# sczhou/CodeFormer

Hardware: NVIDIA H100
Metric: faces_per_sec_512x512_batch32 (higher is better)
Workload: dtype f32 (split-fp16 operands on tensor cores, fp32 accumulate)

## Files before the change

### codeformer_b200/csrc/conv_tc.cu

```cuda

#include <cuda.h>
#include <cuda_fp16.h>
#include <cuda_runtime.h>
#include <stdint.h>

#include <stdlib.h>

#include <atomic>
#include <mutex>

#include "conv_tc.cuh"

namespace cfb {

__global__ void tc_absmax_kernel(const float* __restrict__ w, int64_t total, unsigned* __restrict__ slot) {
  float m = 0.f;
  for (int64_t i = (int64_t)blockIdx.x * blockDim.x + threadIdx.x; i < total; i += (int64_t)gridDim.x * blockDim.x)
    m = fmaxf(m, fabsf(w[i]));
#pragma unroll
  for (int o = 16; o > 0; o >>= 1) m = fmaxf(m, __shfl_xor_sync(0xffffffffu, m, o));
  if ((threadIdx.x & 31) == 0) atomicMax(slot, __float_as_uint(m));
}

__global__ void tc_split_weights_kernel(const float* __restrict__ w, __half* __restrict__ hi, __half* __restrict__ lo,
// ... 221 lines not shown
      else if (clock64() - t0 > *(volatile long long*)&g_wait_limit) { mbar_timeout(); aborted = true; break; }
    }
  }
  aborted = __any_sync(0xffffffffu, aborted);
}
__device__ __forceinline__ void mbar_wait(uint32_t bar, uint32_t parity) {
  uint32_t done = 0;
  const long long t0 = clock64();
  while (!done) {
    asm volatile(
        "{\n\t.reg .pred p;\n\t"
        "mbarrier.try_wait.parity.shared::cta.b64 p, [%1], %2, %3;\n\t"
        "selp.u32 %0, 1, 0, p;\n\t}"
        : "=r"(done)
        : "r"(bar), "r"(parity), "r"(0x989680u)
        : "memory");
    if (!done && clock64() - t0 > *(volatile long long*)&g_wait_limit) { mbar_timeout(); break; }
  }
}
__device__ __forceinline__ void tma_load_4d(uint32_t dst, const CUtensorMap* map, uint32_t bar, int c0, int c1, int c2, int c3) {
  asm volatile(
      "cp.async.bulk.tensor.4d.shared::cluster.global.mbarrier::complete_tx::bytes [%0], [%1, {%3, %4, %5, %6}], [%2];"
      ::"r"(dst), "l"(map), "r"(bar), "r"(c0), "r"(c1), "r"(c2), "r"(c3)
      : "memory");
}
__device__ __forceinline__ void tma_load_3d(uint32_t dst, const CUtensorMap* map, uint32_t bar, int c0, int c1, int c2) {
  asm volatile(
      "cp.async.bulk.tensor.3d.shared::cluster.global.mbarrier::complete_tx::bytes [%0], [%1, {%3, %4, %5}], [%2];"
      ::"r"(dst), "l"(map), "r"(bar), "r"(c0), "r"(c1), "r"(c2)
      : "memory");
}
__device__ __forceinline__ bool elect_one() {
  uint32_t pred;
  asm volatile(
      "{\n\t.reg .b32 rx;\n\t.reg .pred px;\n\t"
      "elect.sync rx|px, 0xffffffff;\n\t"
      "selp.b32 %0, 1, 0, px;\n\t}"
      : "=r"(pred));
  return pred != 0;
}

__device__ __forceinline__ uint64_t wg_desc(uint32_t saddr, uint32_t sbo) {
  return (uint64_t)((saddr >> 4) & 0x3FFFu) | ((uint64_t)1 << 16) | ((uint64_t)((sbo >> 4) & 0x3FFFu) << 32) | ((uint64_t)1 << 62);
}
__device__ __forceinline__ void wg_fence() { asm volatile("wgmma.fence.sync.aligned;" ::: "memory"); }
__device__ __forceinline__ void wg_commit() { asm volatile("wgmma.commit_group.sync.aligned;" ::: "memory"); }
__device__ __forceinline__ void wg_wait_all() { asm volatile("wgmma.wait_group.sync.aligned 0;" ::: "memory"); }
__device__ __forceinline__ void wg_mma_64x64(float (&d)[32], uint64_t da, uint64_t db, uint32_t accum) {
  asm volatile(
      "{\n\t.reg .pred p;\n\t"
      "setp.ne.b32 p, %34, 0;\n\t"
      "wgmma.mma_async.sync.aligned.m64n64k16.f32.f16.f16 "
      "{%0, %1, %2, %3, %4, %5, %6, %7, %8, %9, %10, %11, %12, %13, %14, %15, "
      "%16, %17, %18, %19, %20, %21, %22, %23, %24, %25, %26, %27, %28, %29, %30, %31}, %32, %33, p, 1, 1, 0, 0;\n\t}"
      : "+f"(d[0]), "+f"(d[1]), "+f"(d[2]), "+f"(d[3]), "+f"(d[4]), "+f"(d[5]), "+f"(d[6]), "+f"(d[7]), "+f"(d[8]),
        "+f"(d[9]), "+f"(d[10]), "+f"(d[11]), "+f"(d[12]), "+f"(d[13]), "+f"(d[14]), "+f"(d[15]), "+f"(d[16]),
        "+f"(d[17]), "+f"(d[18]), "+f"(d[19]), "+f"(d[20]), "+f"(d[21]), "+f"(d[22]), "+f"(d[23]), "+f"(d[24]),
        "+f"(d[25]), "+f"(d[26]), "+f"(d[27]), "+f"(d[28]), "+f"(d[29]), "+f"(d[30]), "+f"(d[31])
      : "l"(da), "l"(db), "r"(accum)
      : "memory");
}

__device__ __forceinline__ void wg_mma_64x128(float (&d)[64], uint64_t da, uint64_t db, uint32_t accum) {
  asm volatile(
      "{\n\t.reg .pred p;\n\t"
      "setp.ne.b32 p, %66, 0;\n\t"
      "wgmma.mma_async.sync.aligned.m64n128k16.f32.f16.f16 "
      "{%0, %1, %2, %3, %4, %5, %6, %7, %8, %9, %10, %11, %12, %13, %14, %15, "
      "%16, %17, %18, %19, %20, %21, %22, %23, %24, %25, %26, %27, %28, %29, %30, %31, "
      "%32, %33, %34, %35, %36, %37, %38, %39, %40, %41, %42, %43, %44, %45, %46, %47, "
      "%48, %49, %50, %51, %52, %53, %54, %55, %56, %57, %58, %59, %60, %61, %62, %63}, %64, %65, p, 1, 1, 0, 0;\n\t}"
      : "+f"(d[0]), "+f"(d[1]), "+f"(d[2]), "+f"(d[3]), "+f"(d[4]), "+f"(d[5]), "+f"(d[6]), "+f"(d[7]), "+f"(d[8]),
        "+f"(d[9]), "+f"(d[10]), "+f"(d[11]), "+f"(d[12]), "+f"(d[13]), "+f"(d[14]), "+f"(d[15]), "+f"(d[16]),
        "+f"(d[17]), "+f"(d[18]), "+f"(d[19]), "+f"(d[20]), "+f"(d[21]), "+f"(d[22]), "+f"(d[23]), "+f"(d[24]),
        "+f"(d[25]), "+f"(d[26]), "+f"(d[27]), "+f"(d[28]), "+f"(d[29]), "+f"(d[30]), "+f"(d[31]), "+f"(d[32]),
        "+f"(d[33]), "+f"(d[34]), "+f"(d[35]), "+f"(d[36]), "+f"(d[37]), "+f"(d[38]), "+f"(d[39]), "+f"(d[40]),
        "+f"(d[41]), "+f"(d[42]), "+f"(d[43]), "+f"(d[44]), "+f"(d[45]), "+f"(d[46]), "+f"(d[47]), "+f"(d[48]),
        "+f"(d[49]), "+f"(d[50]), "+f"(d[51]), "+f"(d[52]), "+f"(d[53]), "+f"(d[54]), "+f"(d[55]), "+f"(d[56]),
        "+f"(d[57]), "+f"(d[58]), "+f"(d[59]), "+f"(d[60]), "+f"(d[61]), "+f"(d[62]), "+f"(d[63])
      : "l"(da), "l"(db), "r"(accum)
      : "memory");
}
__device__ __forceinline__ void wg_wait_1() { asm volatile("wgmma.wait_group.sync.aligned 1;" ::: "memory"); }

__device__ __forceinline__ bool wg_any(bool v, uint32_t bar_id = 2) {
  uint32_t r;
  asm volatile(
      "{\n\t.reg .pred p, q;\n\t"
      "setp.ne.u32 p, %1, 0;\n\t"
      "bar.red.or.pred q, %2, 128, p;\n\t"
      "selp.u32 %0, 1, 0, q;\n\t}"
      : "=r"(r)
      : "r"((uint32_t)v), "r"(bar_id)
      : "memory");
  return r != 0;
}

__device__ __forceinline__ float ex2_ftz(float x) { float r; asm("ex2.approx.ftz.f32 %0, %1;" : "=f"(r) : "f"(x)); return r; }
__device__ __forceinline__ float rcp_ftz(float x) { float r; asm("rcp.approx.ftz.f32 %0, %1;" : "=f"(r) : "f"(x)); return r; }
__device__ __forceinline__ uint32_t pack_f16x2(float lo, float hi) {
  uint32_t r;
  asm("cvt.rn.f16x2.f32 %0, %1, %2;" : "=r"(r) : "f"(hi), "f"(lo));
  return r;
}
__device__ __forceinline__ float f16_minus_f32(uint32_t h, float c) {
  return __half2float(__ushort_as_half((unsigned short)h)) - c;
}
__device__ __forceinline__ uint4 lds128(uint32_t addr) {
  uint4 v;
  asm volatile("ld.shared.v4.b32 {%0, %1, %2, %3}, [%4];" : "=r"(v.x), "=r"(v.y), "=r"(v.z), "=r"(v.w) : "r"(addr) : "memory");
  return v;
}
__device__ __forceinline__ void sts128(uint32_t addr, const uint4& v) {
  asm volatile("st.shared.v4.b32 [%0], {%1, %2, %3, %4};" ::"r"(addr), "r"(v.x), "r"(v.y), "r"(v.z), "r"(v.w) : "memory");
}
__device__ __forceinline__ float4 lds128f(uint32_t addr) {
  float4 v;
  asm volatile("ld.shared.v4.f32 {%0, %1, %2, %3}, [%4];" : "=f"(v.x), "=f"(v.y), "=f"(v.z), "=f"(v.w) : "r"(addr));
  return v;
}
__device__ __forceinline__ void sts128f(uint32_t addr, float a, float b, float c, float d) {
  asm volatile("st.shared.v4.f32 [%0], {%1, %2, %3, %4};" ::"r"(addr), "f"(a), "f"(b), "f"(c), "f"(d));
}
template <int MODE, bool LO = true>
__device__ __forceinline__ void xf_chunk(const uint4& a, const uint4& b, const float (&sc)[8], const float (&sh)[8], uint4& hv,
                                         uint4& lv, float& amax) {
  const uint32_t raw[8] = {a.x, a.y, a.z, a.w, b.x, b.y, b.z, b.w};
  uint32_t hw[4], lw[4];
#pragma unroll
  for (int q = 0; q < 4; ++q) {
    float y[2];
#pragma unroll
    for (int e = 0; e < 2; ++e) {
      float v = __uint_as_float(raw[2 * q + e]);
      if (MODE >= 1) v = fmaf(v, sc[2 * q + e], sh[2 * q + e]);
      if (MODE == 2) v = v * rcp_ftz(1.f + ex2_ftz(v * -1.4426950408889634f));
      y[e] = v;
    }
    amax = fmaxf(amax, fmaxf(fabsf(y[0]), fabsf(y[1])));
    hw[q] = pack_f16x2(y[0], y[1]);
    if constexpr (LO) {
      const float d0 = f16_minus_f32(hw[q] & 0xffffu, y[0]);
      const float d1 = f16_minus_f32(hw[q] >> 16, y[1]);
      lw[q] = pack_f16x2(d0, d1) ^ 0x80008000u;
    }
  }
  hv = make_uint4(hw[0], hw[1], hw[2], hw[3]);
  if constexpr (LO) lv = make_uint4(lw[0], lw[1], lw[2], lw[3]);
}
template <int MODE, int RPP, int NPASS, int PW, int ROWS, bool LO = true>
__device__ __forceinline__ void xf_patch(uint32_t src_base, uint32_t hi_base, uint32_t lo_base, int c0, int j, int rsub,
                                         const float (&sc)[8], const float (&sh)[8], bool border, int y0, int x0, int Hin,
                                         int Win, float& amax) {
#pragma unroll
  for (int it = 0; it < NPASS; it += 2) {
    uint4 a[2], b[2];
    bool act[2];
#pragma unroll
    for (int u = 0; u < 2; ++u) {
      const int r = rsub + (it + u) * RPP;
      act[u] = (it + u < NPASS) && (r < ROWS);
      if (act[u]) {
        const uint32_t row = src_base + (uint32_t)r * 128u;
        const uint32_t sw = (row >> 7) & 7u;
        a[u] = lds128(row + (((uint32_t)c0 ^ sw) << 4));
        b[u] = lds128(row + (((uint32_t)(c0 + 1) ^ sw) << 4));
      }
    }
    __syncwarp();
#pragma unroll
    for (int u = 0; u < 2; ++u) {
      if (act[u]) {
        const int r = rsub + (it + u) * RPP;
        uint4 hv, lv;
        xf_chunk<MODE, LO>(a[u], b[u], sc, sh, hv, lv, amax);
        if (border) {
          const int py = r / PW, px = r - py * PW;
          if (!((unsigned)(y0 + py) < (unsigned)Hin && (unsigned)(x0 + px) < (unsigned)Win)) {
            hv = make_uint4(0u, 0u, 0u, 0u);
            if constexpr (LO) lv = make_uint4(0u, 0u, 0u, 0u);
          }
        }
        const uint32_t hrow = hi_base + (uint32_t)r * 128u, lrow = lo_base + (uint32_t)r * 128u;
        sts128(hrow + ((((uint32_t)j) ^ ((hrow >> 7) & 7u)) << 4), hv);
        if constexpr (LO) sts128(lrow + ((((uint32_t)j) ^ ((lrow >> 7) & 7u)) << 4), lv);
      }
    }
    __syncwarp();
  }
}

#ifndef CFB_TC_STAMPS
#define CFB_TC_STAMPS 0
#endif
struct TcParams {
  int N, Ho, Wo, Cout;
  int taps, pad, stride;
  int BW, BH;
  int tiles_x, tiles_y;
  int m_tiles, n_tiles;
  int kblocks;
  int chunk;
  int a_c0, b_c0;
  int b_batched;
  int heads;
  int a_c_head, b_c_head;
  int a_img_per_head;
  int b_r_head;
  int out_per_head;
  int o_c_head;
  int up4;
  int PW, PH;
  int Hin, Win;
  int pad_mode;
  int sub;
  int out_pitch, out_c0, cout_valid;
  int res_pitch;
  const float* residual2;
  int res2_pitch;
  float post_scale;
  int fault;
  int xform;
  int a_split;
  const float* in_scale;
  const float* in_shift;
  int in_act;
  const float* bias;
  const float* residual;
  int out_act;
  const float* sft_dec;
  const float* sft_scale;
  float sft_w;
  const float* wscale_inv;
  float* out;
  __half* pl_hi;
  __half* pl_lo;
  float* gn_part;
  int gn_cpg;
  const float* sft_wv;
#if CFB_TC_STAMPS
  long long* dbg;
#endif
};
#if CFB_TC_STAMPS
#define TC_STAMP(i) do { if (p.dbg != nullptr && blockIdx.x == 0) p.dbg[i] = clock64(); } while (0)
#else
#define TC_STAMP(i) do { } while (0)
#endif

constexpr int XF_SKEW = 128;
constexpr int TC_A_BYTES = 128 * 128;

template <int BN>
struct TcCfg {
  static_assert(BN == 64 || BN == 128, "the wgmma engine runs 64- or 128-wide n-tiles");
  static constexpr bool WIDE = BN == 128;
  static constexpr int MMA_WARPS = WIDE ? 8 : 4;
  static constexpr int EPI_WARPS = WIDE ? 4 : 8;
  static constexpr int THREADS = 32 * (MMA_WARPS + 1 + EPI_WARPS);
  static constexpr int B_BYTES = BN * 128;
  static constexpr int STAGE_BYTES = 2 * TC_A_BYTES + 2 * B_BYTES;
  static constexpr int STAGES = 3;
  static constexpr int SLOT_PITCH = BN + 4;
  static constexpr int SLOT_BYTES = 128 * SLOT_PITCH * 4;
  static constexpr int SLOTS = 1;
  static constexpr int STG_BYTES = WIDE ? 0 : 8 * 4096;
  static constexpr int TAIL_BYTES = SLOT_BYTES + 1024  + 512  + STG_BYTES;
  static constexpr int SMEM_BYTES = STAGES * STAGE_BYTES + TAIL_BYTES;
  static constexpr int H_A_PLANE = 23 * 1024;
  static constexpr int H_A_SLOT = 2 * H_A_PLANE;
  static constexpr int H_A_SLOTS = 2;
  static constexpr int H_B_SLOT = 2 * B_BYTES;
  static constexpr int H_B_SLOTS = WIDE ? 2 : 4;
  static constexpr int H_SMEM_BYTES = H_A_SLOTS * H_A_SLOT + H_B_SLOTS * H_B_SLOT + TAIL_BYTES;
  static constexpr int XF_WARPS = WIDE ? 2 : 4;
  static constexpr int XF_THREADS = THREADS + 32 * XF_WARPS + 32;
  static constexpr int X_A_SLOTS = 2;
  static constexpr int X_A_PLANE2 = H_A_PLANE + XF_SKEW;
  static constexpr int X_B_SLOTS = H_B_SLOTS;
  static constexpr int X_SMEM_BYTES = X_A_SLOTS * H_A_SLOT + X_B_SLOTS * H_B_SLOT + TAIL_BYTES;
};

template <int BN, int CPG, bool HALO, bool XF, bool GEN = false, bool K1 = false, bool CM = false, bool SILU = false,
          bool P1 = false>
__global__ void __launch_bounds__(XF ? TcCfg<BN>::XF_THREADS : TcCfg<BN>::THREADS, 1)
conv_tc_kernel(const __grid_constant__ CUtensorMap tmA_hi, const __grid_constant__ CUtensorMap tmA_lo,
               const __grid_constant__ CUtensorMap tmB_hi, const __grid_constant__ CUtensorMap tmB_lo, const TcParams p) {
  static_assert(!XF || HALO, "the fused operand transform exists for the halo engine only");
  static_assert(!GEN || (XF && CPG == 0), "the generalised addressing exists for the fused-transform engine only");
  static_assert(!K1 || (XF && !GEN && CPG == 0), "K1 = fused transform of a 1x1 conv (patch = tile): its own instantiation");
  using Cfg = TcCfg<BN>;
  constexpr bool WIDE = Cfg::WIDE;
  static_assert(!WIDE || (HALO && !GEN && !K1 && CPG != 2), "128-wide tiles exist for the 3x3 / Upsample halo engine");
  static_assert(!CM || (BN == 64 && HALO && !GEN && !K1), "channel-major tiles exist for the 64-channel 3x3 / Upsample halo convs");
  static_assert(!P1 || (!SILU && !K1 && (GEN || WIDE || CM || !HALO)),
                "the single-pass fp16 variant is built for the generalised, 128-wide, channel-major and per-tap engines");
  constexpr int MMA_WARPS = Cfg::MMA_WARPS, EPI_WARPS = Cfg::EPI_WARPS;
  constexpr int A_SLOTS = XF ? Cfg::X_A_SLOTS : Cfg::H_A_SLOTS;
  constexpr int STAGES = Cfg::STAGES;
  constexpr int STAGE_BYTES = Cfg::STAGE_BYTES;
  const int first_tile = (int)blockIdx.x;
  const int tile_step = (int)gridDim.x;
  extern __shared__ uint8_t smem_raw[];
  uint8_t* smem = reinterpret_cast<uint8_t*>((reinterpret_cast<uintptr_t>(smem_raw) + 1023) & ~(uintptr_t)1023);
  constexpr int NRING = HALO ? (XF ? Cfg::X_B_SLOTS : Cfg::H_B_SLOTS) : STAGES;
  constexpr int RING_BYTES = HALO ? Cfg::H_B_SLOT : STAGE_BYTES;
  uint8_t* ring_base = HALO ? smem + A_SLOTS * Cfg::H_A_SLOT : smem;
  float* acc_slot = reinterpret_cast<float*>(ring_base + NRING * RING_BYTES);
  uint64_t* bars = reinterpret_cast<uint64_t*>(ring_base + NRING * RING_BYTES + Cfg::SLOT_BYTES);
  uint64_t* full = bars;
  uint64_t* empty = bars + NRING;
  uint64_t* cfull = bars + 2 * NRING;
  uint64_t* cempty = bars + 2 * NRING + Cfg::SLOTS;
  uint64_t* afull = bars + 2 * NRING + 2 * Cfg::SLOTS;
  uint64_t* aempty = afull + 3;
  uint64_t* araw = aempty + 3;
  uint8_t* stage_buf = reinterpret_cast<uint8_t*>(bars) + 512;

  constexpr int NWARPS = (XF ? Cfg::XF_THREADS : Cfg::THREADS) / 32;
  const int pwarp = __shfl_sync(0xffffffffu, (int)(threadIdx.x >> 5), 0);
  const int ridx = NWARPS - 1 - pwarp;
  const int warp = pwarp < MMA_WARPS ? 1 : (ridx == 0 ? 0 : ridx + 1);
  const int lane = threadIdx.x & 31;
  bool aborted = false;
  if (threadIdx.x == 0) TC_STAMP(0);

  if (warp == 0 && lane == 0) {
    for (int a = 0; a < 3; ++a) {
      mbar_init(smem_u32(afull + a), XF ? Cfg::XF_WARPS : 1);
      mbar_init(smem_u32(aempty + a), MMA_WARPS);
      mbar_init(smem_u32(araw + a), 1);
    }
    asm volatile("prefetch.tensormap [%0];" ::"l"(&tmA_hi) : "memory");
    asm volatile("prefetch.tensormap [%0];" ::"l"(&tmA_lo) : "memory");
    asm volatile("prefetch.tensormap [%0];" ::"l"(&tmB_hi) : "memory");
    asm volatile("prefetch.tensormap [%0];" ::"l"(&tmB_lo) : "memory");
    for (int s = 0; s < NRING; ++s) { mbar_init(smem_u32(full + s), 1); mbar_init(smem_u32(empty + s), MMA_WARPS); }
    for (int a = 0; a < Cfg::SLOTS; ++a) {
      mbar_init(smem_u32(cfull + a), MMA_WARPS);
      mbar_init(smem_u32(cempty + a), EPI_WARPS);
    }
    asm volatile("fence.mbarrier_init.release.cluster;" ::: "memory");
  }
  __syncthreads();
  pdl_launch_dependents();
  pdl_wait();
  if (threadIdx.x == 0) TC_STAMP(1);

  const int total_tiles = p.m_tiles * p.n_tiles;
  const int nk = p.taps * p.kblocks;

  if (warp == 0) {
    {
      int stage = 0;
      uint32_t phase = 0;
      int aslot = 0;
      uint32_t aphase = 0;
      for (int tile = first_tile; tile < total_tiles; tile += tile_step) {
        const int mt = tile / p.n_tiles, nt = tile - mt * p.n_tiles;
        const int mtl = p.up4 ? (mt >> 2) : mt;
        const int par_y = p.up4 ? ((mt & 3) >> 1) : 0, par_x = p.up4 ? (mt & 1) : 0;
        const int per_img = p.tiles_x * p.tiles_y;
        const int n = mtl / per_img;
        const int rem = mtl - n * per_img;
        const int ty = rem / p.tiles_x, tx = rem - ty * p.tiles_x;
        const int y0 = ty * p.BH * p.stride, x0 = tx * p.BW * p.stride;
        if constexpr (HALO) {
          for (int kb = 0; kb < p.kblocks; ++kb) {
            if constexpr (!XF) {
              mbar_wait<500>(smem_u32(aempty + aslot), aphase ^ 1, aborted); if (aborted) goto teardown;
              if (elect_one()) {
                const uint32_t sa = smem_u32(smem + aslot * Cfg::H_A_SLOT);
                const uint32_t ab = smem_u32(afull + aslot);
                mbar_expect_tx(ab, (uint32_t)((P1 ? 1 : 2) * p.PW * p.PH * 128));
                tma_load_4d(sa, &tmA_hi, ab, kb * 64, x0 - p.pad, y0 - p.pad, n);
                if constexpr (!P1) tma_load_4d(sa + Cfg::H_A_PLANE, &tmA_lo, ab, kb * 64, x0 - p.pad, y0 - p.pad, n);
              }
              __syncwarp();
              if (++aslot == A_SLOTS) { aslot = 0; aphase ^= 1; }
            }
            for (int tap = 0; tap < p.taps; ++tap) {
              const int btap = p.up4 ? (mt & 3) * 4 + tap : tap;
              mbar_wait<500>(smem_u32(empty + stage), phase ^ 1, aborted); if (aborted) goto teardown;
              if (elect_one()) {
                if (tile == first_tile && tap == 0 && kb == 0) TC_STAMP(2);
                const uint32_t sb = smem_u32(ring_base + stage * RING_BYTES);
                const uint32_t fb = smem_u32(full + stage);
                const bool drop = p.fault && blockIdx.x == 0 && tile == first_tile && kb == 0 && tap == 0;
                mbar_expect_tx(fb, (uint32_t)(P1 ? Cfg::B_BYTES : Cfg::H_B_SLOT));
                if (!drop) tma_load_3d(sb, &tmB_hi, fb, kb * 64, nt * BN, btap);
                if constexpr (!P1) tma_load_3d(sb + Cfg::B_BYTES, &tmB_lo, fb, kb * 64, nt * BN, btap);
              }
              __syncwarp();
              if (++stage == NRING) { stage = 0; phase ^= 1; }
            }
          }
        } else {
          for (int tap = 0; tap < p.taps; ++tap) {
            int r, s, btap = tap;
            if (p.up4) { r = (tap >> 1) + par_y; s = (tap & 1) + par_x; btap = (mt & 3) * 4 + tap; }
            else { r = (p.taps == 9) ? tap / 3 : 0; s = (p.taps == 9) ? tap - r * 3 : 0; }
            for (int kb = 0; kb < p.kblocks; ++kb) {
              mbar_wait<500>(smem_u32(empty + stage), phase ^ 1, aborted); if (aborted) goto teardown;
              if (elect_one()) {
                if (tile == first_tile && tap == 0 && kb == 0) TC_STAMP(2);
                const uint32_t sa = smem_u32(smem + stage * STAGE_BYTES);
                const int hh = p.heads > 1 ? n % p.heads : 0, nimg = p.heads > 1 ? n / p.heads : n;
                const int a_img = p.a_img_per_head ? n : nimg;
                const int ac = p.a_c0 + hh * p.a_c_head + kb * 64, bc = p.b_c0 + hh * p.b_c_head + kb * 64;
                const int brow = nt * BN + hh * p.b_r_head;
                const int b3 = p.b_batched ? nimg : btap;
                const uint32_t fb = smem_u32(full + stage);
                const bool drop = p.fault && blockIdx.x == 0 && tile == first_tile && kb == 0 && tap == 0;
                mbar_expect_tx(fb, (uint32_t)(P1 ? TC_A_BYTES + Cfg::B_BYTES : Cfg::STAGE_BYTES));
                tma_load_4d(sa, &tmA_hi, fb, ac, x0 + s - p.pad, y0 + r - p.pad, a_img);
                if constexpr (!P1) tma_load_4d(sa + TC_A_BYTES, &tmA_lo, fb, ac, x0 + s - p.pad, y0 + r - p.pad, a_img);
                if (!drop) tma_load_3d(sa + 2 * TC_A_BYTES, &tmB_hi, fb, bc, brow, b3);
                if constexpr (!P1) tma_load_3d(sa + 2 * TC_A_BYTES + Cfg::B_BYTES, &tmB_lo, fb, bc, brow, b3);
              }
              __syncwarp();
              if (++stage == STAGES) { stage = 0; phase ^= 1; }
            }
          }
        }
      }
    }
  } else if (warp == 1) {
    {
      constexpr bool N128 = WIDE || CM;
      constexpr int MH = N128 ? 1 : 2;
      const uint32_t a_sbo = HALO ? (uint32_t)(p.PW * 128) : 1024u;
      const uint32_t a_half = HALO ? (uint32_t)(8 * p.PW * 128) : 8192u;
      const int wq = (int)(threadIdx.x >> 5) & 3;
      const int wg = (int)(threadIdx.x >> 7);
      const uint32_t bar_id = 2u + (uint32_t)wg;
      const uint32_t slot_base = smem_u32(acc_slot);
      int stage = 0;
      uint32_t phase = 0;
      int slot = 0;
      uint32_t slot_phase = 0;
      int aslot = 0;
      uint32_t aphase = 0;
      float acc[MH][N128 ? 64 : 32];
      if constexpr (N128) {
        for (int tile = first_tile; tile < total_tiles; tile += tile_step) {
          const int par = p.up4 ? ((tile / p.n_tiles) & 3) : 0;
          const int par_y = par >> 1, par_x = par & 1;
          for (int c0 = 0; c0 < nk; c0 += p.chunk) {
            const int c1 = min(c0 + p.chunk, nk);
            uint32_t prev_empty = 0, prev_aempty = 0;
            for (int it = c0; it < c1; ++it) {
              const int kb = it / p.taps;
              const int tap = it - kb * p.taps;
              if (tap == 0) {
                mbar_wait(smem_u32(afull + aslot), aphase, aborted);
                if (wg_any(aborted, bar_id)) { wg_wait_all(); aborted = true; goto teardown; }
              }
              int r = (p.taps == 9) ? tap / 3 : 0;
              int sft = (p.taps == 9) ? tap - r * 3 : 0;
              if (p.up4) { r = (tap >> 1) + par_y; sft = (tap & 1) + par_x; }
              const uint32_t a_hi0 = smem_u32(smem + aslot * Cfg::H_A_SLOT) + (uint32_t)((r * p.PW + sft) * 128) +
                                     (uint32_t)wg * a_half;
              const uint32_t a_lo0 = a_hi0 + (uint32_t)(XF ? Cfg::X_A_PLANE2 : Cfg::H_A_PLANE);
              const uint32_t bsm = smem_u32(ring_base + stage * RING_BYTES);
              mbar_wait(smem_u32(full + stage), phase, aborted);
              if (wg_any(aborted, bar_id)) { wg_wait_all(); aborted = true; goto teardown; }
              wg_fence();
#pragma unroll
              for (int k = 0; k < 4; ++k) {
                const uint64_t db_hi = wg_desc(bsm + 32 * k, 1024u), db_lo = wg_desc(bsm + Cfg::B_BYTES + 32 * k, 1024u);
                const uint64_t da_hi = wg_desc(a_hi0 + 32 * k, a_sbo), da_lo = wg_desc(a_lo0 + 32 * k, a_sbo);
                if constexpr (P1 && CM) {
                  wg_mma_64x128(acc[0], db_hi, da_hi, (it == c0 && k == 0) ? 0u : 1u);
                } else if constexpr (P1) {
                  wg_mma_64x128(acc[0], da_hi, db_hi, (it == c0 && k == 0) ? 0u : 1u);
                } else if constexpr (CM) {
                  wg_mma_64x128(acc[0], db_hi, da_lo, (it == c0 && k == 0) ? 0u : 1u);
                  wg_mma_64x128(acc[0], db_lo, da_hi, 1u);
                  wg_mma_64x128(acc[0], db_hi, da_hi, 1u);
                } else {
                  wg_mma_64x128(acc[0], da_lo, db_hi, (it == c0 && k == 0) ? 0u : 1u);
                  wg_mma_64x128(acc[0], da_hi, db_lo, 1u);
                  wg_mma_64x128(acc[0], da_hi, db_hi, 1u);
                }
              }
              wg_commit();
              wg_wait_1();
              __syncwarp();
              mbar_arrive_if(prev_empty, lane == 0 && prev_empty != 0);
              mbar_arrive_if(prev_aempty, lane == 0 && prev_aempty != 0);
              prev_empty = smem_u32(empty + stage);
              prev_aempty = tap == p.taps - 1 ? smem_u32(aempty + aslot) : 0u;
              if (++stage == NRING) { stage = 0; phase ^= 1; }
              if (tap == p.taps - 1 && ++aslot == A_SLOTS) { aslot = 0; aphase ^= 1; }
            }
            wg_wait_all();
            __syncwarp();
            mbar_arrive_if(prev_empty, lane == 0);
            mbar_arrive_if(prev_aempty, lane == 0 && prev_aempty != 0);
            if constexpr (CM) {
              mbar_wait(smem_u32(cempty + slot), slot_phase ^ 1, aborted);
              if (wg_any(aborted, bar_id)) { aborted = true; goto teardown; }
              const uint32_t st0 = slot_base + (uint32_t)(slot * Cfg::SLOT_BYTES) +
                                   (uint32_t)((2 * (lane & 3) * Cfg::SLOT_PITCH + wq * 16 + (lane >> 2)) * 4);
#pragma unroll
              for (int j = 0; j < 16; ++j) {
#pragma unroll
                for (int h8 = 0; h8 < 2; ++h8) {
#pragma unroll
                  for (int e = 0; e < 2; ++e) {
                    const uint32_t a = st0 + (uint32_t)(((8 * j + e) * Cfg::SLOT_PITCH + 8 * h8) * 4);
                    asm volatile("st.shared.f32 [%0], %1;" ::"r"(a), "f"(acc[0][4 * j + 2 * h8 + e]) : "memory");
                  }
                }
              }
              __syncwarp();
              if (lane == 0) mbar_arrive(smem_u32(cfull + slot));
              if (++slot == Cfg::SLOTS) { slot = 0; slot_phase ^= 1; }
              continue;
            }
            const bool first_chunk = c0 == 0;
            if (first_chunk) {
              mbar_wait(smem_u32(cempty + slot), slot_phase ^ 1, aborted);
              if (wg_any(aborted, bar_id)) { aborted = true; goto teardown; }
            }
            const uint32_t sbase = slot_base + (uint32_t)(slot * Cfg::SLOT_BYTES);
            const int row = wg * 64 + wq * 16 + (lane >> 2);
#pragma unroll
            for (int j = 0; j < 16; ++j) {
#pragma unroll
              for (int h8 = 0; h8 < 2; ++h8) {
                const uint32_t e = sbase + (uint32_t)(((row + 8 * h8) * Cfg::SLOT_PITCH + 8 * j + 2 * (lane & 3)) * 4);
                float x = 0.f, y = 0.f;
                if (!first_chunk) asm volatile("ld.shared.v2.f32 {%0, %1}, [%2];" : "=f"(x), "=f"(y) : "r"(e) : "memory");
                x = __fadd_rn(x, acc[0][4 * j + 2 * h8]);
                y = __fadd_rn(y, acc[0][4 * j + 2 * h8 + 1]);
                asm volatile("st.shared.v2.f32 [%0], {%1, %2};" ::"r"(e), "f"(x), "f"(y) : "memory");
              }
            }
          }
          if constexpr (!CM) {
            __syncwarp();
            if (lane == 0) mbar_arrive(smem_u32(cfull + slot));
            if (++slot == Cfg::SLOTS) { slot = 0; slot_phase ^= 1; }
          }
        }
      } else {
      for (int tile = first_tile; tile < total_tiles; tile += tile_step) {
        const int par = p.up4 ? ((tile / p.n_tiles) & 3) : 0;
        const int par_y = par >> 1, par_x = par & 1;
        for (int it = 0; it < nk; ++it) {
          uint32_t a_hi0, a_lo0, bsm;
          int tap = 0;
          if constexpr (HALO) {
            const int kb = it / p.taps;
            tap = it - kb * p.taps;
            if (tap == 0) { mbar_wait(smem_u32(afull + aslot), aphase, aborted); if (wg_any(aborted)) { aborted = true; goto teardown; } }
            int r = (p.taps == 9) ? tap / 3 : 0;
            int sft = (p.taps == 9) ? tap - r * 3 : 0;
            if (p.up4) { r = (tap >> 1) + par_y; sft = (tap & 1) + par_x; }
            const uint32_t aoff = (uint32_t)((r * p.PW + sft) * 128);
            a_hi0 = smem_u32(smem + aslot * Cfg::H_A_SLOT) + aoff;
            a_lo0 = a_hi0 + (uint32_t)(XF ? Cfg::X_A_PLANE2 : Cfg::H_A_PLANE);
            bsm = smem_u32(ring_base + stage * RING_BYTES);
          } else {
            a_hi0 = smem_u32(smem + stage * STAGE_BYTES);
            a_lo0 = a_hi0 + TC_A_BYTES;
            bsm = a_hi0 + 2 * TC_A_BYTES;
          }
          mbar_wait(smem_u32(full + stage), phase, aborted); if (wg_any(aborted)) { aborted = true; goto teardown; }
          if (blockIdx.x == 0 && threadIdx.x == 0 && tile == first_tile && it == 0) TC_STAMP(3);
          const uint32_t first = (it % p.chunk) == 0 ? 1u : 0u;
          wg_fence();
#pragma unroll
          for (int k = 0; k < 4; ++k) {
            const uint64_t db_hi = wg_desc(bsm + 32 * k, 1024u), db_lo = wg_desc(bsm + Cfg::B_BYTES + 32 * k, 1024u);
#pragma unroll
            for (int mh = 0; mh < 2; ++mh) {
              const uint64_t da_hi = wg_desc(a_hi0 + mh * a_half + 32 * k, a_sbo), da_lo = wg_desc(a_lo0 + mh * a_half + 32 * k, a_sbo);
              if constexpr (P1) {
                wg_mma_64x64(acc[mh], da_hi, db_hi, (first && k == 0) ? 0u : 1u);
              } else {
                wg_mma_64x64(acc[mh], da_lo, db_hi, (first && k == 0) ? 0u : 1u);
                wg_mma_64x64(acc[mh], da_hi, db_lo, 1u);
                wg_mma_64x64(acc[mh], da_hi, db_hi, 1u);
              }
            }
          }
          wg_commit();
          wg_wait_all();
          __syncwarp();
          if (lane == 0) mbar_arrive(smem_u32(empty + stage));
          if (++stage == NRING) { stage = 0; phase ^= 1; }
          if constexpr (HALO) {
            if (tap == p.taps - 1) {
              if (lane == 0) mbar_arrive(smem_u32(aempty + aslot));
              if (++aslot == A_SLOTS) { aslot = 0; aphase ^= 1; }
            }
          }
          if ((it % p.chunk) == p.chunk - 1 || it == nk - 1) {
            mbar_wait(smem_u32(cempty + slot), slot_phase ^ 1, aborted); if (wg_any(aborted)) { aborted = true; goto teardown; }
            const uint32_t sbase = slot_base + (uint32_t)(slot * Cfg::SLOT_BYTES);
#pragma unroll
            for (int mh = 0; mh < 2; ++mh) {
              const int row = mh * 64 + wq * 16 + (lane >> 2);
#pragma unroll
              for (int j = 0; j < 8; ++j) {
                const uint32_t e = sbase + (uint32_t)((row * Cfg::SLOT_PITCH + 8 * j + 2 * (lane & 3)) * 4);
                asm volatile("st.shared.v2.f32 [%0], {%1, %2};" ::"r"(e), "f"(acc[mh][4 * j]), "f"(acc[mh][4 * j + 1]) : "memory");
                asm volatile("st.shared.v2.f32 [%0], {%1, %2};" ::"r"(e + 8 * Cfg::SLOT_PITCH * 4), "f"(acc[mh][4 * j + 2]),
                             "f"(acc[mh][4 * j + 3]) : "memory");
              }
            }
            __syncwarp();
            if (lane == 0) mbar_arrive(smem_u32(cfull + slot));
            if (++slot == Cfg::SLOTS) { slot = 0; slot_phase ^= 1; }
          }
        }
      }
      }
    }
  } else if (XF && warp == 2 + EPI_WARPS + Cfg::XF_WARPS) {
    if constexpr (XF) {
      int aslot = 0;
      uint32_t aphase = 0;
      for (int tile = first_tile; tile < total_tiles; tile += tile_step) {
        const int mt0 = tile / p.n_tiles;
        const int mt = p.up4 ? (mt0 >> 2) : mt0;
        const int per_img = p.tiles_x * p.tiles_y;
        const int n = mt / per_img;
        const int rem = mt - n * per_img;
        const int ty = rem / p.tiles_x, tx = rem - ty * p.tiles_x;
        const int y0 = ty * p.BH, x0 = tx * p.BW;
        for (int kb = 0; kb < p.kblocks; ++kb) {
          mbar_wait<500>(smem_u32(aempty + aslot), aphase ^ 1, aborted); if (aborted) goto teardown;
          if (elect_one()) {
            const uint32_t sa = smem_u32(smem + aslot * Cfg::H_A_SLOT);
            const uint32_t rb = smem_u32(araw + aslot);
            const bool src0 = kb < p.a_split;
            const CUtensorMap* src = src0 ? &tmA_hi : &tmA_lo;
            const int c0 = (src0 ? kb : kb - p.a_split) * 64;
            if (tile == first_tile && kb == 0) TC_STAMP(10);
            mbar_expect_tx(rb, (uint32_t)(2 * p.PW * p.PH * 128));
            tma_load_4d(sa, src, rb, c0, x0 - p.pad, y0 - p.pad, n);
            tma_load_4d(sa + Cfg::X_A_PLANE2, src, rb, c0 + 32, x0 - p.pad, y0 - p.pad, n);
          }
          __syncwarp();
          if (++aslot == A_SLOTS) { aslot = 0; aphase ^= 1; }
        }
      }
    }
  } else if (XF && warp >= 2 + EPI_WARPS) {
    if constexpr (XF) {
      constexpr int XFW = Cfg::XF_WARPS;
      constexpr int RPP = 4 * XFW;
      constexpr int XF_PW = 10, XF_PH = 18, XF_ROWS = XF_PW * XF_PH;
      constexpr int NPASS = (XF_ROWS + RPP - 1) / RPP;
      constexpr int NPASS1 = (128 + RPP - 1) / RPP;
      const int t = (warp - (2 + EPI_WARPS)) * 32 + lane;
      const int j = t & 7, rsub = t >> 3;
      const int pl = j >> 2, c0 = 2 * (j & 3);
      const int mode = p.in_scale ? (p.in_act == IN_SILU ? 2 : 1) : 0;
      const int Hin = GEN ? p.Hin : p.tiles_y * p.BH, Win = GEN ? p.Win : p.tiles_x * p.BW;
      const int Cin = p.kblocks * 64;
      float amax = 0.f;
      int aslot = 0;
      uint32_t aphase = 0;
      for (int tile = first_tile; tile < total_tiles; tile += tile_step) {
        const int mt0 = tile / p.n_tiles;
        const int mt = p.up4 ? (mt0 >> 2) : mt0;
        const int per_img = p.tiles_x * p.tiles_y;
        const int n = mt / per_img;
        const int rem = mt - n * per_img;
        const int ty = rem / p.tiles_x, tx = rem - ty * p.tiles_x;
        const int y0 = ty * p.BH - p.pad, x0 = tx * p.BW - p.pad;
        const bool border = !K1 && (y0 < 0 || x0 < 0 || y0 + XF_PH > Hin || x0 + XF_PW > Win);
        for (int kb = 0; kb < p.kblocks; ++kb) {
          float sc[8], sh[8];
          if (mode) {
            const int nn = GEN ? min(n, p.N - 1) : n;
            const float* sp = p.in_scale + (int64_t)nn * Cin + kb * 64 + j * 8;
            const float* hp = p.in_shift + (int64_t)nn * Cin + kb * 64 + j * 8;
            const float4 s0 = __ldg(reinterpret_cast<const float4*>(sp)), s1 = __ldg(reinterpret_cast<const float4*>(sp + 4));
            const float4 h0 = __ldg(reinterpret_cast<const float4*>(hp)), h1 = __ldg(reinterpret_cast<const float4*>(hp + 4));
            sc[0] = s0.x; sc[1] = s0.y; sc[2] = s0.z; sc[3] = s0.w; sc[4] = s1.x; sc[5] = s1.y; sc[6] = s1.z; sc[7] = s1.w;
            sh[0] = h0.x; sh[1] = h0.y; sh[2] = h0.z; sh[3] = h0.w; sh[4] = h1.x; sh[5] = h1.y; sh[6] = h1.z; sh[7] = h1.w;
          } else {
#pragma unroll
            for (int k = 0; k < 8; ++k) { sc[k] = 1.f; sh[k] = 0.f; }
          }
          mbar_wait<250>(smem_u32(araw + aslot), aphase, aborted); if (aborted) goto teardown;
          if (t == 0 && tile == first_tile && kb == 0) TC_STAMP(11);
          if (t == 0 && tile == first_tile + tile_step && kb == 0) TC_STAMP(19);
          const uint32_t base0 = smem_u32(smem + aslot * Cfg::H_A_SLOT);
          const uint32_t src_base = base0 + (pl ? (uint32_t)Cfg::X_A_PLANE2 : 0u);
          const uint32_t lo_base = base0 + (uint32_t)Cfg::X_A_PLANE2;
          if constexpr (K1) {
            if (mode == 2) xf_patch<2, RPP, NPASS1, 8, 128>(src_base, base0, lo_base, c0, j, rsub, sc, sh, border, y0, x0, Hin, Win, amax);
            else if (mode == 1) xf_patch<1, RPP, NPASS1, 8, 128>(src_base, base0, lo_base, c0, j, rsub, sc, sh, border, y0, x0, Hin, Win, amax);
            else xf_patch<0, RPP, NPASS1, 8, 128>(src_base, base0, lo_base, c0, j, rsub, sc, sh, border, y0, x0, Hin, Win, amax);
          } else {
            if (mode == 2) xf_patch<2, RPP, NPASS, XF_PW, XF_ROWS, !P1>(src_base, base0, lo_base, c0, j, rsub, sc, sh, border, y0, x0, Hin, Win, amax);
            else if (mode == 1) xf_patch<1, RPP, NPASS, XF_PW, XF_ROWS, !P1>(src_base, base0, lo_base, c0, j, rsub, sc, sh, border, y0, x0, Hin, Win, amax);
            else xf_patch<0, RPP, NPASS, XF_PW, XF_ROWS, !P1>(src_base, base0, lo_base, c0, j, rsub, sc, sh, border, y0, x0, Hin, Win, amax);
          }
          if constexpr (GEN) {
            if (p.pad_mode && border) {
              asm volatile("bar.sync 1, %0;" ::"r"(32 * XFW) : "memory");
#pragma unroll 1
              for (int r = rsub; r < XF_ROWS; r += RPP) {
                const int py = r / XF_PW, px = r - py * XF_PW;
                const int gy = y0 + py, gx = x0 + px;
                if ((unsigned)gy < (unsigned)Hin && (unsigned)gx < (unsigned)Win) continue;
                int sy = gy, sx = gx;
                if (p.pad_mode == 1) {
                  sy = sy < 0 ? -sy : (sy >= Hin ? 2 * Hin - 2 - sy : sy);
                  sx = sx < 0 ? -sx : (sx >= Win ? 2 * Win - 2 - sx : sx);
                }
                sy = min(max(sy, max(y0, 0)), min(Hin, y0 + XF_PH) - 1);
                sx = min(max(sx, max(x0, 0)), min(Win, x0 + XF_PW) - 1);
                const int rs = (sy - y0) * XF_PW + (sx - x0);
                const uint32_t hs = base0 + (uint32_t)rs * 128u, hd = base0 + (uint32_t)r * 128u;
                const uint32_t ls = lo_base + (uint32_t)rs * 128u, ld = lo_base + (uint32_t)r * 128u;
                const uint4 hv = lds128(hs + ((((uint32_t)j) ^ ((hs >> 7) & 7u)) << 4));
                if constexpr (P1) {
                  sts128(hd + ((((uint32_t)j) ^ ((hd >> 7) & 7u)) << 4), hv);
                } else {
                  const uint4 lv = lds128(ls + ((((uint32_t)j) ^ ((ls >> 7) & 7u)) << 4));
                  sts128(hd + ((((uint32_t)j) ^ ((hd >> 7) & 7u)) << 4), hv);
                  sts128(ld + ((((uint32_t)j) ^ ((ld >> 7) & 7u)) << 4), lv);
                }
              }
            }
          }
          asm volatile("fence.proxy.async.shared::cta;" ::: "memory");
// ... 63 lines not shown
#pragma unroll
          for (int c0 = 0; c0 < HC; c0 += 4) {
            const float4 v = lds128f(srow + (uint32_t)(c0 * 4));
            acc[c0] += v.x; acc[c0 + 1] += v.y; acc[c0 + 2] += v.z; acc[c0 + 3] += v.w;
          }
          asm volatile("" ::: "memory");
          __syncwarp();
          if (lane == 0) mbar_arrive(smem_u32(cempty + slot));
          if (++slot == Cfg::SLOTS) { slot = 0; slot_phase ^= 1; }
        }
      }
      if (warp == 2 && lane == 0 && tile == first_tile) TC_STAMP(7);
      if (warp == 2 && lane == 0 && tile == first_tile + tile_step) TC_STAMP(17);
      const uint32_t stg = smem_u32(stage_buf) + (uint32_t)(warp - 2) * 4096u;
      const uint32_t stg_w = stg + (uint32_t)lane * 128u;
      const int cch = lane & 7, rsub = lane >> 3;
      if constexpr (GEN) {
        const int Hs = p.sub ? (p.Ho >> 1) : p.Ho, Ws = p.sub ? (p.Wo >> 1) : p.Wo;
#pragma unroll
        for (int q = 0; q < HC; q += 32) {
#pragma unroll
          for (int j = 0; j < 8; ++j)
            sts128f(stg_w + (uint32_t)((j ^ (lane & 7)) << 4), acc[q + 4 * j] * wsi, acc[q + 4 * j + 1] * wsi, acc[q + 4 * j + 2] * wsi,
                    acc[q + 4 * j + 3] * wsi);
          __syncwarp();
          const int colq = col0 + q + cch * 4;
          const bool col_ok = colq < p.cout_valid;
          float4 bv = make_float4(0.f, 0.f, 0.f, 0.f);
          if (p.bias) bv = __ldg(reinterpret_cast<const float4*>(p.bias + colq));
          int64_t pixs[8];
#pragma unroll
          for (int it = 0; it < 8; ++it) {
            const int trow = lg * 32 + it * 4 + rsub;
            const int hh = trow / BW, ww = trow - hh * BW;
            int oy2 = ty * BH + hh, ox2 = tx * BW + ww;
            if (p.up4) { oy2 = 2 * oy2 + ((mt & 3) >> 1); ox2 = 2 * ox2 + (mt & 1); }
            bool ok = col_ok && n < p.N && oy2 < p.Ho && ox2 < p.Wo;
            if (p.sub) { ok = ok && (((oy2 | ox2) & 1) == 0); oy2 >>= 1; ox2 >>= 1; }
            pixs[it] = ok ? ((int64_t)n * Hs + oy2) * Ws + ox2 : (int64_t)-1;
          }
          float4 rres[8];
#pragma unroll
          for (int it = 0; it < 8; ++it)
            rres[it] = (p.residual && pixs[it] >= 0) ? __ldg(reinterpret_cast<const float4*>(p.residual + pixs[it] * p.res_pitch + colq))
                                                     : make_float4(0.f, 0.f, 0.f, 0.f);
#pragma unroll
          for (int it = 0; it < 8; ++it) {
            const int r = it * 4 + rsub;
            float4 v = lds128f(stg + (uint32_t)(r * 128 + ((cch ^ (r & 7)) << 4)));
            v.x += bv.x + rres[it].x; v.y += bv.y + rres[it].y; v.z += bv.z + rres[it].z; v.w += bv.w + rres[it].w;
            if (p.out_act == OUT_LRELU || p.out_act == OUT_RELU) {
              const float sl = p.out_act == OUT_LRELU ? 0.2f : 0.f;
              v.x = v.x > 0.f ? v.x : sl * v.x; v.y = v.y > 0.f ? v.y : sl * v.y;
              v.z = v.z > 0.f ? v.z : sl * v.z; v.w = v.w > 0.f ? v.w : sl * v.w;
            } else if (SILU) {
              v.x = tc_silu_out(v.x); v.y = tc_silu_out(v.y); v.z = tc_silu_out(v.z); v.w = tc_silu_out(v.w);
            }
            if (pixs[it] >= 0) {
              if (p.residual2) {
                const float4 r2 = __ldg(reinterpret_cast<const float4*>(p.residual2 + pixs[it] * p.res2_pitch + colq));
                v.x = fmaf(v.x, p.post_scale, r2.x); v.y = fmaf(v.y, p.post_scale, r2.y);
                v.z = fmaf(v.z, p.post_scale, r2.z); v.w = fmaf(v.w, p.post_scale, r2.w);
              }
              *reinterpret_cast<float4*>(p.out + pixs[it] * p.out_pitch + p.out_c0 + colq) = v;
            }
          }
          __syncwarp();
        }
      } else {
      const uint32_t slot_q = smem_u32(acc_slot) + (uint32_t)(slot * Cfg::SLOT_BYTES) +
                              (uint32_t)(((lg * 32 + rsub) * Cfg::SLOT_PITCH + cbase + cch * 4) * 4);
#pragma unroll
      for (int q = 0; q < HC; q += 32) {
        if constexpr (!WIDE) {
#pragma unroll
          for (int j = 0; j < 8; ++j)
            sts128f(stg_w + (uint32_t)((j ^ (lane & 7)) << 4), acc[q + 4 * j] * wsi, acc[q + 4 * j + 1] * wsi, acc[q + 4 * j + 2] * wsi,
                    acc[q + 4 * j + 3] * wsi);
          __syncwarp();
        }
        const int colq = col0 + q + cch * 4;
        float4 bv = make_float4(0.f, 0.f, 0.f, 0.f);
        if (p.bias) bv = __ldg(reinterpret_cast<const float4*>(p.bias + colq));
        constexpr int RB = (XF && !WIDE) ? 4 : 8;
        float s0 = 0.f, q0 = 0.f, s1 = 0.f, q1 = 0.f, k0 = 0.f, k1 = 0.f;
#pragma unroll
        for (int ib = 0; ib < 8; ib += RB) {
        int64_t offs[RB];
        bool inside[RB];
#pragma unroll
        for (int k = 0; k < RB; ++k) {
          const int it = ib + k;
          const int trow = lg * 32 + it * 4 + rsub;
          const int hh = bw_shift >= 0 ? (trow >> bw_shift) : trow / BW, ww = trow - hh * BW;
          offs[k] = off_tile + colq + hh * SH + ww * SW;
          inside[k] = whole_tiles || ((ty * BH + hh) * ts < p.Ho && (tx * BW + ww) * ts < p.Wo);
        }
        float4 rres[RB];
#pragma unroll
        for (int k = 0; k < RB; ++k)
          rres[k] = (p.residual && inside[k]) ? __ldg(reinterpret_cast<const float4*>(p.residual + offs[k])) : make_float4(0.f, 0.f, 0.f, 0.f);
#pragma unroll
        for (int k = 0; k < RB; ++k) {
          const int it = ib + k;
          const int r = it * 4 + rsub;
          float4 v;
          if constexpr (WIDE) {
            v = lds128f(slot_q + (uint32_t)((it * 4 * Cfg::SLOT_PITCH + q) * 4));
            v.x = __fmul_rn(v.x, wsi); v.y = __fmul_rn(v.y, wsi); v.z = __fmul_rn(v.z, wsi); v.w = __fmul_rn(v.w, wsi);
          } else {
            v = lds128f(stg + (uint32_t)(r * 128 + ((cch ^ (r & 7)) << 4)));
          }
          const int64_t off = offs[k];
          v.x += bv.x + rres[k].x; v.y += bv.y + rres[k].y; v.z += bv.z + rres[k].z; v.w += bv.w + rres[k].w;
          if (p.out_act == OUT_LRELU) {
            v.x = v.x > 0.f ? v.x : 0.2f * v.x; v.y = v.y > 0.f ? v.y : 0.2f * v.y;
            v.z = v.z > 0.f ? v.z : 0.2f * v.z; v.w = v.w > 0.f ? v.w : 0.2f * v.w;
          } else if (p.out_act == OUT_GELU) {
            v.x = 0.5f * v.x * (1.f + erff(v.x * 0.70710678118654752440f));
            v.y = 0.5f * v.y * (1.f + erff(v.y * 0.70710678118654752440f));
            v.z = 0.5f * v.z * (1.f + erff(v.z * 0.70710678118654752440f));
            v.w = 0.5f * v.w * (1.f + erff(v.w * 0.70710678118654752440f));
          } else if (p.out_act == OUT_RELU) {
            v.x = fmaxf(v.x, 0.f); v.y = fmaxf(v.y, 0.f); v.z = fmaxf(v.z, 0.f); v.w = fmaxf(v.w, 0.f);
          } else if (SILU) {
            v.x = tc_silu_out(v.x); v.y = tc_silu_out(v.y); v.z = tc_silu_out(v.z); v.w = tc_silu_out(v.w);
          }
          if (p.sft_dec && inside[k]) {
            const float4 d = __ldg(reinterpret_cast<const float4*>(p.sft_dec + off));
            const float4 sc = __ldg(reinterpret_cast<const float4*>(p.sft_scale + off));
            float sw = p.sft_w;
            if constexpr (!XF) { if (p.sft_wv) { const float t = __ldg(p.sft_wv + n); sw = t > 0.f ? t : 0.f; } }
            v.x = d.x + sw * (d.x * sc.x + v.x); v.y = d.y + sw * (d.y * sc.y + v.y);
            v.z = d.z + sw * (d.z * sc.z + v.z); v.w = d.w + sw * (d.w * sc.w + v.w);
          }
          if (!inside[k]) v = make_float4(0.f, 0.f, 0.f, 0.f);
          if (p.out && inside[k]) *reinterpret_cast<float4*>(p.out + off) = v;
          if (p.pl_hi && inside[k]) {
            omax = fmaxf(omax, fmaxf(fmaxf(fabsf(v.x), fabsf(v.y)), fmaxf(fabsf(v.z), fabsf(v.w))));
            const __half2 h01 = __floats2half2_rn(v.x, v.y), h23 = __floats2half2_rn(v.z, v.w);
            const float2 f01 = __half22float2(h01), f23 = __half22float2(h23);
            const __half2 l01 = __floats2half2_rn(v.x - f01.x, v.y - f01.y), l23 = __floats2half2_rn(v.z - f23.x, v.w - f23.y);
            uint2 ph, pl;
            ph.x = *reinterpret_cast<const uint32_t*>(&h01); ph.y = *reinterpret_cast<const uint32_t*>(&h23);
            pl.x = *reinterpret_cast<const uint32_t*>(&l01); pl.y = *reinterpret_cast<const uint32_t*>(&l23);
            *reinterpret_cast<uint2*>(p.pl_hi + off) = ph;
            *reinterpret_cast<uint2*>(p.pl_lo + off) = pl;
          }
          if constexpr (CPG == 2) {
            if (it == 0) { k0 = v.x; k1 = v.z; }
            const float a = v.x - k0, b = v.y - k0, c = v.z - k1, d = v.w - k1;
            s0 += a + b; q0 += fmaf(a, a, b * b);
            s1 += c + d; q1 += fmaf(c, c, d * d);
          } else if constexpr (CPG >= 4) {
            if (it == 0) k0 = v.x;
            const float a = v.x - k0, b = v.y - k0, c = v.z - k0, d = v.w - k0;
            s0 += (a + b) + (c + d);
            q0 += fmaf(a, a, b * b) + fmaf(c, c, d * d);
          }
        }
        }
        if constexpr (CPG > 0) {
          constexpr float NL = CPG == 2 ? 16.f : 32.f;
          gn_lane_moments(s0, q0, k0, NL);
          if constexpr (CPG == 2) gn_lane_moments(s1, q1, k1, NL);
          gn_merge_xor(s0, q0, 8, NL); gn_merge_xor(s0, q0, 16, 2.f * NL);
          if constexpr (CPG == 2) { gn_merge_xor(s1, q1, 8, NL); gn_merge_xor(s1, q1, 16, 2.f * NL); }
// ... 824 lines not shown
```

Before: 174.5.

## Rebalance registers via setmaxnreg and defer accumulator hand-off in wide tiles

For the 128-wide tile engine, thread count is padded to 512 so setmaxnreg can move registers from producer and epilogue warpgroups (down to 96) to the MMA warpgroups (up to 160). The MMA warps now keep a running fp32 sum of the chunk accumulators in registers instead of read-modify-writing shared memory per chunk. The finished tile is stored to the slot only after the next tile's first wgmma has been issued, so the store overlaps tensor-core work. This costs extra register pressure (64 more live floats) and idle pad warps, and the epilogue row batch and transform-loop unroll factors are also changed.

After: 189.9, median of 6. +8.8%, better.

```diff
diff --git a/codeformer_b200/csrc/conv_tc.cu b/codeformer_b200/csrc/conv_tc.cu
--- a/codeformer_b200/csrc/conv_tc.cu
+++ b/codeformer_b200/csrc/conv_tc.cu
@@ -327,6 +327,8 @@
       : "memory");
 }
 __device__ __forceinline__ void wg_wait_1() { asm volatile("wgmma.wait_group.sync.aligned 1;" ::: "memory"); }
+template <int N> __device__ __forceinline__ void wg_regs_inc() { asm volatile("setmaxnreg.inc.sync.aligned.u32 %0;" ::"n"(N)); }
+template <int N> __device__ __forceinline__ void wg_regs_dec() { asm volatile("setmaxnreg.dec.sync.aligned.u32 %0;" ::"n"(N)); }
 
 __device__ __forceinline__ bool wg_any(bool v, uint32_t bar_id = 2) {
   uint32_t r;
@@ -397,7 +399,7 @@
 __device__ __forceinline__ void xf_patch(uint32_t src_base, uint32_t hi_base, uint32_t lo_base, int c0, int j, int rsub,
                                          const float (&sc)[8], const float (&sh)[8], bool border, int y0, int x0, int Hin,
                                          int Win, float& amax) {
-#pragma unroll
+#pragma unroll (RPP >= 16 ? 64 : 1)
   for (int it = 0; it < NPASS; it += 2) {
     uint4 a[2], b[2];
     bool act[2];
@@ -502,7 +504,7 @@
   static constexpr bool WIDE = BN == 128;
   static constexpr int MMA_WARPS = WIDE ? 8 : 4;
   static constexpr int EPI_WARPS = WIDE ? 4 : 8;
-  static constexpr int THREADS = 32 * (MMA_WARPS + 1 + EPI_WARPS);
+  static constexpr int THREADS = WIDE ? 512 : 32 * (MMA_WARPS + 1 + EPI_WARPS);
   static constexpr int B_BYTES = BN * 128;
   static constexpr int STAGE_BYTES = 2 * TC_A_BYTES + 2 * B_BYTES;
   static constexpr int STAGES = 3;
@@ -519,7 +521,8 @@
   static constexpr int H_B_SLOTS = WIDE ? 2 : 4;
   static constexpr int H_SMEM_BYTES = H_A_SLOTS * H_A_SLOT + H_B_SLOTS * H_B_SLOT + TAIL_BYTES;
   static constexpr int XF_WARPS = WIDE ? 2 : 4;
-  static constexpr int XF_THREADS = THREADS + 32 * XF_WARPS + 32;
+  static constexpr int XF_THREADS = 32 * (MMA_WARPS + 1 + EPI_WARPS + XF_WARPS + 1);
+  static_assert(!WIDE || XF_THREADS == THREADS, "the 128-wide transform variant fills the pad warps exactly");
   static constexpr int X_A_SLOTS = 2;
   static constexpr int X_A_PLANE2 = H_A_PLANE + XF_SKEW;
   static constexpr int X_B_SLOTS = H_B_SLOTS;
@@ -568,6 +571,9 @@
   const int warp = pwarp < MMA_WARPS ? 1 : (ridx == 0 ? 0 : ridx + 1);
   const int lane = threadIdx.x & 31;
   bool aborted = false;
+  if constexpr (WIDE) {
+    if (pwarp >= MMA_WARPS) wg_regs_dec<96>();
+  }
   if (threadIdx.x == 0) TC_STAMP(0);
 
   if (warp == 0 && lane == 0) {
@@ -671,6 +677,7 @@
       }
     }
   } else if (warp == 1) {
+    if constexpr (WIDE) wg_regs_inc<160>();
     {
       constexpr bool N128 = WIDE || CM;
       constexpr int MH = N128 ? 1 : 2;
@@ -688,6 +695,28 @@
       uint32_t aphase = 0;
       float acc[MH][N128 ? 64 : 32];
       if constexpr (N128) {
+        float run[64];
+        auto hand_off = [&]() -> bool {
+          mbar_wait(smem_u32(cempty + slot), slot_phase ^ 1, aborted);
+          if (wg_any(aborted, bar_id)) return true;
+          const int row = wg * 64 + wq * 16 + (lane >> 2);
+          uint32_t e0;
+          asm volatile("mov.b32 %0, %1;" : "=r"(e0)
+                       : "r"(slot_base + (uint32_t)(slot * Cfg::SLOT_BYTES) + (uint32_t)((row * Cfg::SLOT_PITCH + 2 * (lane & 3)) * 4)));
+#pragma unroll
+          for (int j = 0; j < 16; ++j) {
+#pragma unroll
+            for (int h8 = 0; h8 < 2; ++h8) {
+              const uint32_t e = e0 + (uint32_t)((8 * h8 * Cfg::SLOT_PITCH + 8 * j) * 4);
+              asm volatile("st.shared.v2.f32 [%0], {%1, %2};" ::"r"(e), "f"(run[4 * j + 2 * h8]), "f"(run[4 * j + 2 * h8 + 1])
+                           : "memory");
+            }
+          }
+          __syncwarp();
+          if (lane == 0) mbar_arrive(smem_u32(cfull + slot));
+          if (++slot == Cfg::SLOTS) { slot = 0; slot_phase ^= 1; }
+          return false;
+        };
         for (int tile = first_tile; tile < total_tiles; tile += tile_step) {
           const int par = p.up4 ? ((tile / p.n_tiles) & 3) : 0;
           const int par_y = par >> 1, par_x = par & 1;
@@ -730,6 +759,11 @@
                 }
               }
               wg_commit();
+              if constexpr (WIDE) {
+                if (it == 0 && tile != first_tile) {
+                  if (hand_off()) { wg_wait_all(); aborted = true; goto teardown; }
+                }
+              }
               wg_wait_1();
               __syncwarp();
               mbar_arrive_if(prev_empty, lane == 0 && prev_empty != 0);
@@ -764,31 +798,14 @@
               if (++slot == Cfg::SLOTS) { slot = 0; slot_phase ^= 1; }
               continue;
             }
-            const bool first_chunk = c0 == 0;
-            if (first_chunk) {
-              mbar_wait(smem_u32(cempty + slot), slot_phase ^ 1, aborted);
-              if (wg_any(aborted, bar_id)) { aborted = true; goto teardown; }
+            if constexpr (WIDE) {
+#pragma unroll
+              for (int i = 0; i < 64; ++i) run[i] = __fadd_rn(c0 == 0 ? 0.f : run[i], acc[0][i]);
             }
-            const uint32_t sbase = slot_base + (uint32_t)(slot * Cfg::SLOT_BYTES);
-            const int row = wg * 64 + wq * 16 + (lane >> 2);
-#pragma unroll
-            for (int j = 0; j < 16; ++j) {
-#pragma unroll
-              for (int h8 = 0; h8 < 2; ++h8) {
-                const uint32_t e = sbase + (uint32_t)(((row + 8 * h8) * Cfg::SLOT_PITCH + 8 * j + 2 * (lane & 3)) * 4);
-                float x = 0.f, y = 0.f;
-                if (!first_chunk) asm volatile("ld.shared.v2.f32 {%0, %1}, [%2];" : "=f"(x), "=f"(y) : "r"(e) : "memory");
-                x = __fadd_rn(x, acc[0][4 * j + 2 * h8]);
-                y = __fadd_rn(y, acc[0][4 * j + 2 * h8 + 1]);
-                asm volatile("st.shared.v2.f32 [%0], {%1, %2};" ::"r"(e), "f"(x), "f"(y) : "memory");
-              }
-            }
-          }
-          if constexpr (!CM) {
-            __syncwarp();
-            if (lane == 0) mbar_arrive(smem_u32(cfull + slot));
-            if (++slot == Cfg::SLOTS) { slot = 0; slot_phase ^= 1; }
-          }
+          }
+        }
+        if constexpr (WIDE) {
+          if (first_tile < total_tiles && hand_off()) { aborted = true; goto teardown; }
         }
       } else {
       for (int tile = first_tile; tile < total_tiles; tile += tile_step) {
@@ -895,7 +912,8 @@
         }
       }
     }
-  } else if (XF && warp >= 2 + EPI_WARPS) {
+  } else if ((XF || WIDE) && warp >= 2 + EPI_WARPS) {
+
     if constexpr (XF) {
       constexpr int XFW = Cfg::XF_WARPS;
       constexpr int RPP = 4 * XFW;
@@ -1125,7 +1143,7 @@
         const int colq = col0 + q + cch * 4;
         float4 bv = make_float4(0.f, 0.f, 0.f, 0.f);
         if (p.bias) bv = __ldg(reinterpret_cast<const float4*>(p.bias + colq));
-        constexpr int RB = (XF && !WIDE) ? 4 : 8;
+        constexpr int RB = (XF || WIDE) ? 4 : 8;
         float s0 = 0.f, q0 = 0.f, s1 = 0.f, q1 = 0.f, k0 = 0.f, k1 = 0.f;
 #pragma unroll
         for (int ib = 0; ib < 8; ib += RB) {
```
